# Nick-qsv/MLP-PPO-2PLY-MULTI

Measured on AMD Instinct MI355X. Metric: self-play env steps/sec (whole node) at 1-ply and 2-ply, 1/2/4/8 MI355X, higher is better.
Workload: dtype u8 game state + fp16x2-split MFMA (fp32 acc); 1 GPU; 8192 game lanes per GPU (8192 total), 1-ply softmax select (configs[3]/[4] lane shard: 65,536 lanes at N=8); lanes_per_gpu=8192, lanes_total=8192, ply=1, harvest_every=300, engine=fused step kernel, lockstep launches (reproducible: --dump-outputs), parallelism=single GPU

## Files before the change

### mlp-ppo-2ply-multi_amd/csrc/bgx_fused.hip

```cpp
#define BGX_LANE_ID_AT_USE 1
#include "bgx_engine.h"
#include "bgx_mlp.h"
#include "bgx_movegen.h"

namespace bgx {

constexpr int PROF_STRIDE = 128;

template <int FL> struct FusedTail {
    uint4 lut[256];
    float w2s[128];
    int cnt[FL];
    int go[2];
    int qn[2];
    int ncl;
    unsigned tdone[64];
    unsigned chosen[FL];
    unsigned claim[FL];
    int pre[FL + 1];
    uint32_t job[FL][8];
    DrawSlot draw[FL];
    LaneState st[FL];
};
template <int FL> struct FCfg {
    static constexpr int NW = 12;
    static constexpr int WPE = NW / 4;
    static constexpr int P1_S = 256, P1_F = 160, P1_PF = 416;
    static constexpr int SL1 = 64 * 4 + 2 * P1_PF * 4;
    static constexpr int F_SCR = NW * SL1 > Slice<S_T2>::bytes ? NW * SL1 : Slice<S_T2>::bytes;
    static constexpr int F_W = F_SCR;
    static constexpr int CP_F = 128 * NW;
    static_assert(sizeof(CoopPathLds<NW, CP_F>) <= F_SCR, "path expansion fits the scratch");
    static constexpr int F_TAIL = F_W + NFRAG * 16;
    static constexpr int XS_FIT = (160 * 1024 - F_TAIL - (int)sizeof(FusedTail<FL>)) / (FL * 4);
    static constexpr int XS = XS_FIT < 96 ? XS_FIT : 96;
    static constexpr int LDS = F_TAIL + (int)sizeof(FusedTail<FL>) + FL * XS * 4;
    static_assert(XS >= 24 && LDS <= 160 * 1024, "fits the CU's LDS");
};

__device__ __forceinline__ const FusedArgs& launch_args() {
    auto p = __builtin_amdgcn_kernarg_segment_ptr();
    asm volatile("" : "+s"(p));
    return *(const FusedArgs*)p;
}
__device__ __forceinline__ MovegenArgs job_args(const FusedArgs& f) {
    MovegenArgs a{};
    a.out_mode = OUT_PACKED_SLOT;
    a.cap = f.cap;
    a.out_packed = f.cand;
    a.out_count = const_cast<int32_t*>(f.e.cand_cnt);
    a.ws_global = f.ws_global;
    a.ws_slots = f.ws_slots;
    a.ws_words_per_wave = f.ws_words_per_block;
    a.force_tier = f.force_tier;
    a.err_flags = f.e.err_flags;
    return a;
}

template <bool PROF, int FL>
__global__ __launch_bounds__(64 * FCfg<FL>::NW, FCfg<FL>::WPE) void fused_step_kernel(FusedArgs) {
    using C = FCfg<FL>;
    constexpr int NW = C::NW, SL1 = C::SL1, F_W = C::F_W, F_TAIL = C::F_TAIL, XS = C::XS;
    constexpr int P1_S = C::P1_S, P1_F = C::P1_F, P1_PF = C::P1_PF;
    constexpr int CP_F = C::CP_F;
    constexpr bool PAIR = FL == 32;
    constexpr int NT = 64 * NW;
    extern __shared__ __attribute__((aligned(16))) unsigned long long smem[];
    uint8_t* lds = (uint8_t*)smem;
    FusedTail<FL>& T = *(FusedTail<FL>*)(lds + F_TAIL);
    float* xs = (float*)(lds + F_TAIL + sizeof(FusedTail<FL>));
    const int t = (int)threadIdx.x, w = t >> 6, l = lane_id();
    {
        const FusedArgs& f = launch_args();
        for (int i = t; i < 256; i += NT) T.lut[i] = lut_entry((uint32_t)i, f.feat_scale);
        for (int i = t; i < 128; i += NT) T.w2s[i] = f.rowc[i];
    }
    for (int i = t; i < 64; i += NT) T.tdone[i] = 0u;
    for (int i = t; i < FL; i += NT) T.chosen[i] = T.claim[i] = 0u;
    unsigned qtag = 0u;
    uint4* wl = (uint4*)(lds + F_W);
    static_assert(NFRAG % 64 == 0, "W fragments in whole wave chunks");
    {
        const uint4* const wsrc = launch_args().wfrag;
        for (int c = w; c < NFRAG / 64; c += NW)
            __builtin_amdgcn_global_load_lds((__attribute__((address_space(1))) void*)(void*)(wsrc + 64 * c + l),
                                             (__attribute__((address_space(3))) void*)(void*)(wl + 64 * c), 16, 0, 0);
    }
    const uint4* wf = wl;

    unsigned long long n_rows = 0, n_fb = 0, n_steps = 0;
    const unsigned long long wg_begin = PROF ? wall_clock64() : 0ull;
    const unsigned long long cyc_begin = PROF ? __builtin_amdgcn_s_memtime() : 0ull;
    unsigned long long t_loop0 = 0, t_loop1 = 0;
    unsigned long long t_step = 0, late_sum = 0, late_n = 0;
    int step_idx = 0;
    unsigned long long ph[6] = {0, 0, 0, 0, 0, 0}, tc = 0, tw[4] = {0, 0, 0, 0}, t2c = 0, t3n = 0;
    unsigned long long tjd[4] = {0, 0, 0, 0};
    unsigned long long tcs[3] = {0, 0, 0};
    unsigned long long tdr[3] = {0, 0, 0};
    unsigned long long tms[3] = {0, 0, 0};
    unsigned long long tpr[7] = {0, 0, 0, 0, 0, 0, 0};
    constexpr bool prof = PROF;
    auto tick = [&](int k) {
        if (prof && t == 0) {
            const unsigned long long c = wall_clock64();
            ph[k] += c - tc;
            tc = c;
        }
    };
    const int groups = (launch_args().e.L + FL - 1) / FL;
    uint32_t* const slw = (uint32_t*)(lds + (size_t)w * SL1);
    Mem M1 = slice_mem<P1_S, P1_F, P1_PF>(slw);
    asm volatile("s_waitcnt vmcnt(0)" ::: "memory");
    for (int g = (int)blockIdx.x; g < groups; g += (int)gridDim.x) {
        int nlive, n_iter;
        bool t1_ready;
        {
            const FusedArgs& f = launch_args();
            nlive = f.e.L - g * FL < FL ? f.e.L - g * FL : FL;
            n_iter = f.budget > 0 ? f.n_cap : f.n_steps;
            t1_ready = f.t1_ready != 0;
            for (int v = t; v < nlive; v += NT) {
                lane_load(f.e, g * FL + v, T.st[v]);
                if (t1_ready) T.cnt[v] = f.t1cnt[g * FL + v];
            }
        }
        if (t1_ready) {
            __syncthreads();
            for (int q = t; q < nlive * 8; q += NT) {
                const int v = q >> 3, k = q & 7;
                const LaneState& st = T.st[v];
                T.job[v][k] = k < 7 ? st.w[k] : (uint32_t)st.p | ((uint32_t)st.d0 << 8) | ((uint32_t)st.d1 << 16);
            }
        }
        auto ticket = [&](int s) -> int {
            const FusedArgs& f = launch_args();
            const int full = nlive << 8;
            if (f.budget <= 0) return s < f.n_steps ? full : 0;
            if (s >= f.n_cap) return 0;
            const unsigned long long old = atomicAdd(f.budget_ctr, (unsigned long long)nlive);
            return old < (unsigned long long)f.budget ? full : 0;
        };
        auto wait_flag = [&](const unsigned* fl) {
            for (unsigned spin = 0; __hip_atomic_load(fl, __ATOMIC_RELAXED, __HIP_MEMORY_SCOPE_WORKGROUP) != qtag;
                 ++spin) {
                if (spin >= (1u << 24)) {
                    if (l == 0) atomicOr(launch_args().e.err_flags, BGX_ERRF_WAIT_BOUND);
                    break;
                }
                __builtin_amdgcn_s_sleep(1);
            }
        };
        if (prof && t == 0 && !t_loop0) t_loop0 = wall_clock64();
        for (int step = -1; step < n_iter; ++step) {
            int nr = 0;
            const int gv = step >= 0 ? T.go[step & 1] : nlive << 8;
            if (!gv) break;
            const int lo = gv & 255, hi = gv >> 8;
            const auto act = [&](int v) { return v >= lo && v < hi; };
            if (prof && t == 0) tc = wall_clock64();
            if (step >= 0) {
                n_steps += (unsigned long long)(hi - lo);
                const int cnt_l = act(l) ? T.cnt[l] : 0;
                uint32_t ovf = (uint32_t)ballot(l < FL && cnt_l < 0);
                while (ovf) {
                    const int v = __ffs(ovf) - 1;
                    ovf &= ovf - 1u;
                    ++n_fb;
                    const unsigned long long c2 = prof ? wall_clock64() : 0ull;
                    const int j = g * FL + v;
                    const uint32_t* q = T.job[v];
                    const JobIn in = make_job(q[0], q[1], q[2], q[3], q[4], q[5], q[6], (int)(q[7] & 255u),
                                              (int)((q[7] >> 8) & 255u), (int)(q[7] >> 16));
                    const FusedArgs& f = launch_args();
                    const MovegenArgs a = job_args(f);
                    FlatCursor fc;
                    auto run_global = [&]() -> int {
                        uint32_t* base = f.ws_global + (size_t)blockIdx.x * f.ws_words_per_block;
                        const Mem G = global_mem(base, f.ws_slots);
                        st32<true>(G.map + l, 0u);
                        sync<true>();
                        if (prof) ++t3n;
                        const int r = run_job<true>(a, j, in, G, fc);
                        if (r < 0 && l == 0) atomicOr(a.err_flags, BGX_ERRF_FALLBACK_OVERFLOW);
                        return r < 0 ? 0 : r;
                    };
                    int r2 = -1;
                    if (in.d0 == in.d1 && doubles_by_path(in.R) && f.force_tier < 3) {
                        auto& C = *(CoopPathLds<NW, CP_F>*)lds;
                        uint32_t* fin = nullptr;
                        r2 = coop_doubles_path<NW, CP_F>(in, C, fin);
                        if (r2 >= 0) {
                            emit_records<false>(a, j, in, fin, r2, 0, 64 * w, 64 * NW);
                            if (t == 0) {
                                T.cnt[v] = r2;
                                a.out_count[j] = r2;
                            }
                        }
                        __syncthreads();
                    }
                    if (r2 < 0 && w == 0) {
                        const Mem M2 = lds_mem<S_T2>(smem);
                        int r = f.force_tier >= 3 ? -1 : run_job<false>(a, j, in, M2, fc);
                        if (r < 0) r = run_global();
                        if (l == 0) T.cnt[v] = r;
                    }
                    __syncthreads();
                    if (prof) t2c += wall_clock64() - c2;
                }
                const int c = act(l) ? T.cnt[l] : 0;
                const int cap = launch_args().cap;
                const int rows = l < FL && c > 0 ? 1 + (c < cap ? c : cap) : 0;
                const int incl = wave_incl_scan(rows);
                if (l <= FL) T.pre[l] = incl - rows;
                wave_sync();
                nr = T.pre[FL];
                n_rows += (unsigned long long)nr;
                tick(1);
            }
            const int n_tiles = (nr + 31) >> 5;
            const int np = step >= 0 ? (hi - lo + 1) >> 1 : 0;
            if (t == 0) {
                T.qn[0] = NW;
                T.qn[1] = NW;
                T.ncl = 0;
            }
            ++qtag;
            M1.map[l] = 0u;
            wave_sync();
            __syncthreads();
            const int nj = step >= 0 || !t1_ready ? hi - lo : 0;
            const bool dbl = act(l) && T.st[l].d0 == T.st[l].d1;
            const uint32_t dmask = (uint32_t)ballot(dbl), omask = (uint32_t)ballot(act(l) && !dbl);
            const int nd = __popc(dmask);
            auto lane_of = [&](int r) -> int {
                int v = 0;
#pragma unroll
                for (int sstep = FL / 2; sstep >= 1; sstep >>= 1)
                    if (T.pre[v + sstep] <= r) v += sstep;
                return v;
            };
            const unsigned long long m0 = prof ? wall_clock64() : 0ull;
            const bool one = n_tiles <= 64;
            const int npass = one ? 1 : 3;
            for (int pass = 0; pass < npass; ++pass) {
                const int qt = one || pass == 0 ? n_tiles : 0;
                const int qp = one || pass == 1 ? np : 0;
                const int qj = one || pass == 2 ? nj : 0;
                const bool pipelined = one && np > 0;
                int* qc = &T.qn[pass & 1];
                const int qd = pass == npass - 1 ? 1 : 0;
                int it = w;
                while (it < qt + qp + qj + qd) {
                    if (it < qt) {
                        const unsigned long long i0 = prof ? wall_clock64() : 0ull;
                        const FusedArgs& f = launch_args();
                        const uint32_t* const k_rows = f.e.rows;
                        const uint32_t* const k_cand = f.cand;
                        float* const k_vbuf = f.vbuf;
                        const int k_cap = f.cap;
                        const float k_b2 = f.b2, k_fs = f.feat_scale;
                        const int r = it * 32 + (l & 31);
                        uint4 bx = make_uint4(0, 0, 0, 0), by = make_uint4(0, 0, 0, 0);
                        int vl = 0, k = 0;
                        if (r < nr) {
                            vl = lane_of(r);
                            k = r - T.pre[vl];
                            const int li = g * FL + vl;
                            const uint32_t* src =
                                k == 0 ? k_rows + (size_t)li * 8 : k_cand + ((size_t)li * k_cap + (k - 1)) * 8;
                            bx = ((const uint4*)src)[0];
                            by = ((const uint4*)src)[1];
                        }
                        unsigned long long i1 = 0, i2 = 0;
                        if (prof) {
                            __builtin_amdgcn_s_waitcnt(0);
                            i1 = wall_clock64();
                            tms[0] += i1 - i0;
                        }
                        const float v = mlp_tile4<PROF>(wf, T.lut, T.w2s, k_fs, bx, by, &i2);
                        if (prof) {
                            const float vv = __shfl(v, 0);
                            asm volatile("" ::"v"(vv));
                            const unsigned long long i3 = wall_clock64();
                            tms[1] += i2 - i1;
                            tms[2] += i3 - i2;
                        }
                        if (l < 32 && r < nr) {
                            const float val = v + k_b2;
                            if (k < XS) xs[vl * XS + k] = val;
                            else k_vbuf[(size_t)(g * FL + vl) * (k_cap + 1) + k] = val;
                        }
                        __builtin_amdgcn_fence(__ATOMIC_RELEASE, "workgroup");
                        if (l == 0) __hip_atomic_store(&T.tdone[it & 63], qtag, __ATOMIC_RELAXED, __HIP_MEMORY_SCOPE_WORKGROUP);
                        if (prof) tw[1] += wall_clock64() - i0;
                    } else if (it < qt + qp) {
                        const int p = it - qt;
                        const FusedArgs& f = launch_args();
                        const EngineDev& e = f.e;
                        if (pipelined) {
                            const int va = lo + 2 * p, vb = lo + 2 * p + 2 < hi ? lo + 2 * p + 2 : hi;
                            const int r0 = T.pre[va], r1 = T.pre[vb];
                            if (r1 > r0) {
                                for (int tt = r0 >> 5; tt <= (r1 - 1) >> 5; ++tt) wait_flag(&T.tdone[tt]);
                                __builtin_amdgcn_fence(__ATOMIC_ACQUIRE, "workgroup");
                            }
                        }
                        const int v = lo + 2 * p + (l >> 5);
                        const bool lead = (l & 31) == 0;
                        if (v < hi) {
                            const int i = g * FL + v;
                            const unsigned long long s1 = prof ? wall_clock64() : 0ull;
                            LaneState sr = T.st[v];
                            const int n_full = T.cnt[v];
                            const int n = n_full < e.max_legal ? n_full : e.max_legal;
                            SlotRng rng;
                            rng.seed = e.seed;
                            rng.gid = (uint32_t)(e.lane_base + i);
                            rng.dt = lane_dice(e, i);
                            rng.load(T.draw[v], sr.ctr);
                            unsigned long long c0 = 0;
                            if (prof) {
                                __builtin_amdgcn_s_waitcnt(0);
                                c0 = wall_clock64();
                                tcs[0] += c0 - s1;
                            }
                            if (n <= 0) {
                                lane_advance(e, i, sr, rng, -1, sr.w, 0.0f, 0.0f, 0, lead);
                            } else {
                                const float* xv = xs + v * XS;
                                const float* vv = f.vbuf + (size_t)i * (f.cap + 1);
                                const float Tm = e.temperature;
                                const float u = rng.uniform01();
                                const int pick =
                                    n + 1 <= XS
                                        ? pick_action_half([&](int kk) { return xv[1 + kk] / Tm; }, n, e.greedy != 0, u)
                                        : pick_action_half(
                                              [&](int kk) { return (1 + kk < XS ? xv[1 + kk] : vv[1 + kk]) / Tm; }, n,
                                              e.greedy != 0, u);
                                if (prof) {
                                    const unsigned long long c1 = wall_clock64();
                                    tw[2] += c1 - s1;
                                    tcs[1] += c1 - c0;
                                    c0 = c1;
                                }
                                uint32_t nb[8];
                                load_packed(f.cand + ((size_t)i * f.cap + pick) * 8, nb);
                                const float va = 1 + pick < XS ? xv[1 + pick] : vv[1 + pick];
                                lane_advance(e, i, sr, rng, pick, nb, xv[0], va, n_full, lead);
                                if (prof) {
                                    __builtin_amdgcn_s_waitcnt(0);
                                    tcs[2] += wall_clock64() - c0;
                                }
                            }
                            wave_sync();
                            if (lead) T.st[v] = sr;
                            if (prof) tw[3] += wall_clock64() - s1;
                        }
                        __builtin_amdgcn_fence(__ATOMIC_RELEASE, "workgroup");
                        if (lead && v < hi)
                            __hip_atomic_store(&T.chosen[v], qtag, __ATOMIC_RELAXED, __HIP_MEMORY_SCOPE_WORKGROUP);
                    } else if (it < qt + qp + qj) {
                        const int kj = it - qt - qp;
                        const FusedArgs& f = launch_args();
                        const MovegenArgs a = job_args(f);
                        const bool k_pair = f.pair != 0;
                        int v, v2 = -1;
                        if (pipelined) {
                            v = -1;
                            for (unsigned spin = 0; v < 0; ++spin) {
                                const bool ready =
                                    act(l) &&
                                    __hip_atomic_load(&T.chosen[l], __ATOMIC_RELAXED, __HIP_MEMORY_SCOPE_WORKGROUP) == qtag &&
                                    __hip_atomic_load(&T.claim[l], __ATOMIC_RELAXED, __HIP_MEMORY_SCOPE_WORKGROUP) != qtag;
                                __builtin_amdgcn_fence(__ATOMIC_ACQUIRE, "workgroup");
                                const bool isd = ready && T.st[l].d0 == T.st[l].d1;
                                const uint32_t md = (uint32_t)ballot(isd), mo = (uint32_t)ballot(ready && !isd);
                                if (md | mo) {
                                    const int cand = md ? __ffs(md) - 1 : __ffs(mo) - 1;
                                    int won = 0;
                                    if (l == 0) {
                                        const unsigned old = T.claim[cand];
                                        won = old != qtag && atomicCAS(&T.claim[cand], old, qtag) == old;
                                        if (PAIR && won) atomicAdd(&T.ncl, 1);
                                    }
                                    if (uniform(won)) v = cand;
                                    if (prof && v >= 0) tpr[2] += 1;
                                } else {
                                    if (PAIR &&
                                        uniform(__hip_atomic_load(&T.ncl, __ATOMIC_RELAXED, __HIP_MEMORY_SCOPE_WORKGROUP)) >= nj)
                                        break;
                                    if (spin >= (1u << 24)) {
                                        if (l == 0) atomicOr(a.err_flags, BGX_ERRF_WAIT_BOUND);
                                        v = kj;
                                        break;
                                    }
                                    __builtin_amdgcn_s_sleep(1);
                                }
                            }
                        } else {
                            v = kj < nd ? select_bit(dmask, kj) : select_bit(omask, kj - nd);
                        }
                        if (PAIR && pipelined && v >= 0 && (k_pair || prof) && T.st[v].d0 != T.st[v].d1) {
                            const bool free_l =
                                act(l) &&
                                __hip_atomic_load(&T.chosen[l], __ATOMIC_RELAXED, __HIP_MEMORY_SCOPE_WORKGROUP) == qtag &&
                                __hip_atomic_load(&T.claim[l], __ATOMIC_RELAXED, __HIP_MEMORY_SCOPE_WORKGROUP) != qtag;
                            __builtin_amdgcn_fence(__ATOMIC_ACQUIRE, "workgroup");
                            const bool cls = (free_l || l == v) && T.st[l].d0 != T.st[l].d1 &&
                                             nd_by_rule(make_root(T.st[l].w, (int)T.st[l].p));
                            const uint32_t mc = (uint32_t)ballot(cls);
                            uint32_t mf = mc & ~(1u << v);
                            if ((mc >> v) & 1u) {
                                if (prof) {
                                    tpr[3] += 1;
                                    if (mf) tpr[4] += 1;
                                }
                                for (int att = 0; att < 2 && mf && v2 < 0 && k_pair; ++att) {
                                    const int c2 = __ffs(mf) - 1;
                                    mf &= mf - 1u;
                                    int won2 = 0;
                                    if (l == 0) {
                                        const unsigned old = T.claim[c2];
                                        won2 = old != qtag && atomicCAS(&T.claim[c2], old, qtag) == old;
                                        if (won2) atomicAdd(&T.ncl, 1);
                                    }
                                    if (uniform(won2)) v2 = c2;
                                }
                            }
                        }
                        const unsigned long long q0 = prof ? wall_clock64() : 0ull;
                        bool paired = false;
                        if (PAIR && v2 >= 0) {
                            if (l < 16) {
                                const int vq = l < 8 ? v : v2, k = l & 7;
                                const LaneState& sq = T.st[vq];
                                T.job[vq][k] =
                                    k < 7 ? sq.w[k] : (uint32_t)sq.p | ((uint32_t)sq.d0 << 8) | ((uint32_t)sq.d1 << 16);
                            }
                            wave_sync();
                            int na = 0, nb = 0;
                            paired = a.force_tier < 2 &&
                                     job_records_pair<false>(a, g * FL + v, T.job[v], g * FL + v2, T.job[v2], M1, na, nb);
                            wave_sync();
                            if (paired && l == 0) {
                                T.cnt[v] = na;
                                T.cnt[v2] = nb;
                            }
                            if (prof && paired) {
                                tpr[5] += wall_clock64() - q0;
                                tpr[6] += 1;
                            }
                        }
                        const int nv = !PAIR ? 1 : (v < 0 ? 0 : (v2 >= 0 ? 2 : 1));
                        for (int q = 0; q < nv; ++q) {
                            const int vq = q ? v2 : v;
                            const unsigned long long q1 = prof ? wall_clock64() : 0ull;
                            const LaneState& st = T.st[vq];
                            if (l < 8)
                                T.job[vq][l] =
                                    l < 7 ? st.w[l] : (uint32_t)st.p | ((uint32_t)st.d0 << 8) | ((uint32_t)st.d1 << 16);
                            if (paired) continue;
                            const JobIn in =
                                make_job(st.w[0], st.w[1], st.w[2], st.w[3], st.w[4], st.w[5], st.w[6], st.p, st.d0, st.d1);
                            int rule2 = 0;
                            uint32_t* fin = nullptr;
                            const int nf = a.force_tier >= 2
                                               ? -1
                                               : job_records<false>(in, M1, fin, prof ? &rule2 : nullptr);
                            if (nf >= 0) emit_records<false>(a, g * FL + vq, in, fin, nf, 0);
                            wave_sync();
                            if (l == 0) T.cnt[vq] = nf;
                            if (prof) {
                                const int kd = in.d0 == in.d1 ? 0 : 2;
                                tjd[kd] += wall_clock64() - q1;
                                tjd[kd + 1] += 1;
                                if (rule2) {
                                    tpr[0] += wall_clock64() - q1;
                                    tpr[1] += 1;
                                }
                            }
                        }
                    } else {
                        const unsigned long long d0 = prof ? wall_clock64() : 0ull;
                        const FusedArgs& f = launch_args();
                        const int ld = lane_id();
                        const int v = ld & (FL - 1), k = ld / FL;
                        const bool mine = k < 2 && act(v);
                        if (pipelined) {
                            for (unsigned spin = 0;; ++spin) {
                                const bool pend =
                                    mine &&
                                    __hip_atomic_load(&T.chosen[v], __ATOMIC_RELAXED, __HIP_MEMORY_SCOPE_WORKGROUP) != qtag;
                                if (!ballot(pend)) break;
                                if (spin >= (1u << 24)) {
                                    if (l == 0) atomicOr(f.e.err_flags, BGX_ERRF_WAIT_BOUND);
                                    break;
                                }
                                __builtin_amdgcn_s_sleep(1);
                            }
                            __builtin_amdgcn_fence(__ATOMIC_ACQUIRE, "workgroup");
                        }
                        const unsigned long long d1 = prof ? wall_clock64() : 0ull;
                        if (mine)
                            draw_fill(T.draw[v], f.e.seed, (uint32_t)(f.e.lane_base + g * FL + v), T.st[v].ctr, k);
                        if (prof) {
                            __builtin_amdgcn_s_waitcnt(0);
                            tdr[0] += wall_clock64() - d0;
                            tdr[1] += d1 - d0;
                            tdr[2] += 1;
                        }
                    }
                    int kn = 0;
                    if (l == 0) kn = atomicAdd(qc, 1);
                    it = uniform(kn);
                }
                if (pass + 1 < npass) {
                    if (t == 0) T.qn[(pass + 1) & 1] = NW;
                    __syncthreads();
                }
            }
            if (prof) tw[0] += wall_clock64() - m0;
            tick(3);
            if (t == 0) T.go[(step + 1) & 1] = ticket(step + 1);
            __syncthreads();
            tick(4);
            if (prof && t == 0 && step >= 0) ph[5] += 1;
            if (prof && t == 0) {
                const unsigned long long c = wall_clock64();
                if (step >= 0) {
                    if (step_idx < 24) {
                        unsigned long long* const pr = launch_args().prof;
                        atomicAdd(pr + (size_t)blockIdx.x * PROF_STRIDE + 32 + step_idx, c - t_step);
                        atomicAdd(pr + (size_t)blockIdx.x * PROF_STRIDE + 64 + step_idx, 1ull);
                    }
                    else { late_sum += c - t_step; ++late_n; }
                    ++step_idx;
                }
                t_step = c;
            }
        }
        if (prof && t == 0) t_loop1 = wall_clock64();
        const FusedArgs& f = launch_args();
        const EngineDev& e = f.e;
        for (int v = t; v < nlive; v += NT) {
            lane_store(e, g * FL + v, T.st[v]);
            f.t1cnt[g * FL + v] = T.cnt[v];
        }
        if (f.hv_hdr) {
            uint32_t* hs = (uint32_t*)lds;
            if (w == 0) {
                int ne = 0, nr = 0;
                bool lost = false;
                if (l < nlive) {
                    const LaneState& s = T.st[l];
                    ne = (int)(s.epi - s.hepi);
                    nr = (int)(s.ep_first - s.harv);
                    lost = ne > e.HR || nr > e.R;
                }
                if (lost) ne = nr = 0;
                const int ie = wave_incl_scan(ne), ir = wave_incl_scan(nr);
                const uint32_t te = (uint32_t)__shfl(ie, 63), tr = (uint32_t)__shfl(ir, 63);
                if (l < FL) {
                    hs[l] = (uint32_t)(ie - ne);
                    hs[64 + l] = (uint32_t)(ir - nr);
                }
                if (l == 0) {
                    unsigned long long base = 0ull;
                    uint32_t fit = 1u;
                    if (te | tr) {
                        const unsigned long long add = ((unsigned long long)te << 32) | tr;
                        base = atomicAdd(f.hv_ctr, add);
                        fit = (base >> 32) + te <= (unsigned long long)f.hv_ep_cap &&
                              (base & 0xFFFFFFFFull) + tr <= (unsigned long long)f.hv_rec_cap;
                        if (fit) atomicAdd(f.hv_commit, add);
                    }
                    hs[128] = te;
                    hs[129] = tr;
                    hs[130] = (uint32_t)(base >> 32);
                    hs[131] = (uint32_t)base;
                    hs[132] = fit;
                }
                if (l < FL) hs[136 + l] = lost ? 1u : 0u;
            }
            __syncthreads();
            const uint32_t te = hs[128], tr = hs[129], be = hs[130], br = hs[131], fit = hs[132];
            auto owner = [&](const uint32_t* pre, uint32_t k) -> int {
                int v = 0;
#pragma unroll
                for (int sstep = FL / 2; sstep >= 1; sstep >>= 1)
                    if (pre[v + sstep] <= k) v += sstep;
                return v;
            };
            if (fit) {
                for (uint32_t q = (uint32_t)t; q < 4u * te; q += NT) {
                    const uint32_t k = q >> 2;
                    const int v = owner(hs, k);
                    const uint32_t ep = T.st[v].hepi + (k - hs[v]);
                    const uint4* src = (const uint4*)(e.hring + ((size_t)(g * FL + v) * e.HR + (ep & (uint32_t)(e.HR - 1))) *
                                                                    EP_WORDS);
                    ((uint4*)(f.hv_hdr + (size_t)(be + k) * EP_WORDS))[q & 3u] = src[q & 3u];
                }
                for (uint32_t q = (uint32_t)t; q < 3u * tr; q += NT) {
                    const uint32_t r = q / 3u, c = q - 3u * r;
                    const int v = owner(hs + 64, r);
                    const uint32_t rr = T.st[v].harv + (r - hs[64 + v]);
                    const uint4* src =
                        (const uint4*)(e.ring + ((size_t)(g * FL + v) * e.R + (rr & (uint32_t)(e.R - 1))) * REC_WORDS);
                    ((uint4*)(f.hv_rec + (size_t)(br + r) * REC_WORDS))[c] = src[c];
                }
            }
            for (int v = t; v < nlive; v += NT) {
                if (fit || hs[136 + v]) {
                    e.harv[g * FL + v] = T.st[v].ep_first;
                    e.hepi[g * FL + v] = T.st[v].epi;
                }
            }
        }
        __syncthreads();
    }
    const FusedArgs& f = launch_args();
    const EngineDev& e = f.e;
    if (prof) {
        unsigned long long* P = f.prof + (size_t)blockIdx.x * PROF_STRIDE;
        if (t == 0) {
            P[24] = wg_begin;
            P[25] = wall_clock64();
            P[26] = n_rows;
            P[27] = n_fb;
            P[28] = n_steps;
            P[19] = t_loop0;
            P[20] = t_loop1;
            P[21] = __builtin_amdgcn_s_memtime() - cyc_begin;
            for (int k = 0; k < 6; ++k) atomicAdd(P + k, ph[k]);
            atomicAdd(P + 11, t2c);
            atomicAdd(P + 12, n_fb);
            atomicAdd(P + 13, t3n);
            atomicAdd(P + 18, (unsigned long long)NW * ph[5]);
            atomicAdd(P + 56, late_sum);
            atomicAdd(P + 57, late_n);
        }
        if (l == 0) {
            for (int k = 0; k < 4; ++k) atomicAdd(P + 7 + k, tw[k]);
            for (int k = 0; k < 4; ++k) atomicAdd(P + 14 + k, tjd[k]);
            for (int k = 0; k < 3; ++k) atomicAdd(P + 29 + k, tcs[k]);
            atomicAdd(P + 6, tms[0]);
            atomicAdd(P + 22, tms[1]);
            atomicAdd(P + 23, tms[2]);
            for (int k = 0; k < 7; ++k) atomicAdd(P + 88 + k, tpr[k]);
            for (int k = 0; k < 3; ++k) atomicAdd(P + 95 + k, tdr[k]);
        }
    }
    if (t == 0) {
        atomicAdd(e.stats + 0, n_steps);
        atomicAdd(e.stats + 3, n_rows);
        atomicAdd(e.stats + 4, n_steps);
        atomicAdd(e.stats + 5, n_fb);
        if (f.budget > 0 || f.hv_hdr) {
            __builtin_amdgcn_fence(__ATOMIC_RELEASE, "agent");
            if (atomicAdd(f.done_ctr, 1ull) == (unsigned long long)gridDim.x - 1ull) {
                __builtin_amdgcn_fence(__ATOMIC_ACQUIRE, "agent");
                if (f.budget > 0) __hip_atomic_store(f.budget_ctr, 0ull, __ATOMIC_RELAXED, __HIP_MEMORY_SCOPE_AGENT);
                if (f.hv_hdr) {
                    const unsigned long long c = __hip_atomic_load(f.hv_commit, __ATOMIC_RELAXED, __HIP_MEMORY_SCOPE_AGENT);
                    const uint32_t fl = atomicExch(e.err_flags, 0u) | (uint32_t)*f.hv_flags;
                    *f.hv_flags = fl;
                    *f.hv_next_flags = 0ull;
                    const uint32_t v[4] = {(uint32_t)(c >> 32), (uint32_t)c, fl, (uint32_t)(c >> 32)};
#pragma unroll
                    for (int k = 0; k < 4; ++k) {
                        f.hv_info[k] = v[k];
                        if (f.hv_hinfo) f.hv_hinfo[k] = v[k];
                    }
                    __hip_atomic_store(f.hv_next, 0ull, __ATOMIC_RELAXED, __HIP_MEMORY_SCOPE_AGENT);
                    __hip_atomic_store(f.hv_next_commit, 0ull, __ATOMIC_RELAXED, __HIP_MEMORY_SCOPE_AGENT);
                }
                __hip_atomic_store(f.done_ctr, 0ull, __ATOMIC_RELAXED, __HIP_MEMORY_SCOPE_AGENT);
            }
        }
    }
}

}

#ifdef BGX_STAMP
extern "C" int bgx_diag_stamps(unsigned long long* out32) {
    static unsigned long long h[256 * 32];
    if (hipMemcpyFromSymbol(h, HIP_SYMBOL(bgx::bgx_stamp_acc), sizeof(h)) != hipSuccess) return -1;
    for (int k = 0; k < 32; ++k) {
        out32[k] = 0;
        for (int b = 0; b < 256; ++b) out32[k] += h[b * 32 + k];
    }
    static unsigned long long z[256 * 32];
    return hipMemcpyToSymbol(HIP_SYMBOL(bgx::bgx_stamp_acc), z, sizeof(z)) == hipSuccess ? 0 : -1;
}
#endif

extern "C" hipError_t bgx_launch_fused(const bgx::FusedArgs* args, hipStream_t stream) {
    static int n_cu_dev[64] = {0};
    int cur = 0;
    if (hipGetDevice(&cur) != hipSuccess || cur < 0 || cur >= 64) cur = 0;
    int& n_cu = n_cu_dev[cur];
    if (!n_cu) {
        if (hipDeviceGetAttribute(&n_cu, hipDeviceAttributeMultiprocessorCount, cur) != hipSuccess || n_cu <= 0)
            n_cu = 256;
        const void* k16[] = {(const void*)bgx::fused_step_kernel<false, 16>, (const void*)bgx::fused_step_kernel<true, 16>};
        const void* k32[] = {(const void*)bgx::fused_step_kernel<false, 32>, (const void*)bgx::fused_step_kernel<true, 32>};
        for (const void* k : k16)
            if (hipFuncSetAttribute(k, hipFuncAttributeMaxDynamicSharedMemorySize, bgx::FCfg<16>::LDS) != hipSuccess)
                return hipErrorInvalidValue;
        for (const void* k : k32)
            if (hipFuncSetAttribute(k, hipFuncAttributeMaxDynamicSharedMemorySize, bgx::FCfg<32>::LDS) != hipSuccess)
                return hipErrorInvalidValue;
    }
    if (args->n_steps <= 0 || args->e.L <= 0) return hipSuccess;
    if (args->cap < 1 || args->cap > 2048) return hipErrorInvalidValue;
    const int L = args->e.L;
    const int fl = args->lanes_per_wg == 16 || args->lanes_per_wg == 32 ? args->lanes_per_wg
                   : ((L + 31) / 32 >= n_cu ? 32 : 16);
    const int groups = (L + fl - 1) / fl;
    int blocks = groups < n_cu ? groups : n_cu;
    if (blocks > args->ws_blocks) blocks = args->ws_blocks;
    const dim3 g(blocks), b(64 * (fl == 32 ? bgx::FCfg<32>::NW : bgx::FCfg<16>::NW));
    bgx::FusedArgs a = *args;
    if (a.budget > 0 && (groups > blocks || !a.budget_ctr || a.n_cap < a.n_steps)) a.budget = 0;
    if (fl == 32) {
        if (a.prof)
            hipLaunchKernelGGL((bgx::fused_step_kernel<true, 32>), g, b, bgx::FCfg<32>::LDS, stream, a);
        else
            hipLaunchKernelGGL((bgx::fused_step_kernel<false, 32>), g, b, bgx::FCfg<32>::LDS, stream, a);
    } else {
        if (a.prof)
            hipLaunchKernelGGL((bgx::fused_step_kernel<true, 16>), g, b, bgx::FCfg<16>::LDS, stream, a);
        else
            hipLaunchKernelGGL((bgx::fused_step_kernel<false, 16>), g, b, bgx::FCfg<16>::LDS, stream, a);
    }
    return hipGetLastError();
}
```

### mlp-ppo-2ply-multi_amd/csrc/bgx_host_prof.cpp

```cpp
#include "bgx_prof.h"

#include <algorithm>
#include <utility>
#include <vector>

void fused_prof_report(const unsigned long long* p, int n_slots, FILE* out, const char* dump_path) {
    constexpr size_t W = kProfSlotWords;
    double s[W] = {0};
    for (int b = 0; b < n_slots; ++b)
        for (size_t k = 0; k < W; ++k) s[k] += (double)p[(size_t)b * W + k];
    const double n = s[5] > 0 ? s[5] : 1;
    const double nws = s[18] > 0 ? s[18] : 1;
    fprintf(out, "[bgx fused prof] us per workgroup step: tier2 + prefix %.2f, queue %.2f, end barrier %.2f "
            "(%.0f workgroup steps)\n", s[1] / n / 100, s[3] / n / 100, s[4] / n / 100, n);
    fprintf(out, "[bgx fused prof] wave-us per workgroup step in items: MLP tiles %.2f, choice pairs %.2f, "
            "tier-1 jobs %.2f (%.2f per wave-step of %d waves)\n", s[8] / n / 100, s[10] / n / 100,
            (s[14] + s[16]) / n / 100, (s[8] + s[10] + s[14] + s[16]) / nws / 100, (int)(nws / n + 0.5));
    fprintf(out, "[bgx fused prof] choice per wave-step: state + Philox refill %.2f, pick %.2f, "
            "env step %.2f us\n", s[29] / nws / 100, s[30] / nws / 100, s[31] / nws / 100);
    fprintf(out, "[bgx fused prof] draw item: %.2f us each, %.2f of it waiting for the choices (%.0f items, "
            "%.2f per workgroup step)\n", s[95] / (s[97] > 0 ? s[97] : 1) / 100,
            s[96] / (s[97] > 0 ? s[97] : 1) / 100, s[97], s[97] / n);
    fprintf(out, "[bgx fused prof] MLP tiles per workgroup step: rows + k mask %.2f, MFMA chain issue %.2f, "
            "drain + epilogue %.2f wave-us\n", s[6] / n / 100, s[22] / n / 100, s[23] / n / 100);
    fprintf(out, "[bgx fused prof] step us by index in the launch (workgroup-steps):");
    for (int k = 0; k < 24; ++k)
        fprintf(out, " %.2f (%.0f)", s[64 + k] > 0 ? s[32 + k] / s[64 + k] / 100 : 0.0, s[64 + k]);
    fprintf(out, "; later steps %.2f (%.0f)\n", s[57] > 0 ? s[56] / s[57] / 100 : 0.0, s[57]);
    fprintf(out, "[bgx fused prof] tier-2 jobs %.0f (%.0f reached tier 3), %.1f us each\n", s[12], s[13],
            s[11] / (s[12] > 0 ? s[12] : 1) / 100);
    fprintf(out, "[bgx fused prof] tier-1 job: doubles %.2f us (%.0f jobs), non-doubles %.2f us (%.0f jobs)\n",
            s[14] / (s[15] > 0 ? s[15] : 1) / 100, s[15], s[16] / (s[17] > 0 ? s[17] : 1) / 100, s[17]);
    const double items = s[8] + s[10] + s[14] + s[16] + s[93];
    fprintf(out, "[bgx fused prof] tier-1 rule-mode two-move job: %.2f us (%.0f jobs), %.2f wave-us per workgroup "
            "step, %.1f %% of the item wave-us\n", s[88] / (s[89] > 0 ? s[89] : 1) / 100, s[89], s[88] / n / 100,
            100.0 * s[88] / (items > 0 ? items : 1));
    fprintf(out, "[bgx fused prof] pipelined job claims %.0f: %.0f of a rule-mode non-doubles lane, %.0f of them "
            "(%.1f %%) with a second such lane ready and unclaimed\n", s[90], s[91], s[92],
            100.0 * s[92] / (s[91] > 0 ? s[91] : 1));
    fprintf(out, "[bgx fused prof] tier-1 pair items: %.0f pairs formed (%.2f per workgroup step), %.2f us each, "
            "%.2f wave-us per workgroup step\n", s[94], s[94] / n, s[93] / (s[94] > 0 ? s[94] : 1) / 100,
            s[93] / n / 100);
    std::vector<std::pair<double, int>> dur;
    unsigned long long b_min = ~0ull, b_max = 0, e_max = 0;
    for (int b = 0; b < n_slots; ++b) {
        const unsigned long long* q = &p[(size_t)b * W];
        if (q[25] <= q[24]) continue;
        dur.push_back({(double)(q[25] - q[24]) / 100.0, b});
        b_min = q[24] < b_min ? q[24] : b_min;
        b_max = q[24] > b_max ? q[24] : b_max;
        e_max = q[25] > e_max ? q[25] : e_max;
    }
    if (dump_path) {
        if (FILE* fp = fopen(dump_path, "w")) {
            fprintf(fp, "wg,begin,end,loop0,loop1,rows,tier2,lane_steps\n");
            for (int b = 0; b < n_slots; ++b) {
                const unsigned long long* q = &p[(size_t)b * W];
                if (q[25] <= q[24]) continue;
                fprintf(fp, "%d,%llu,%llu,%llu,%llu,%llu,%llu,%llu\n", b, q[24], q[25], q[19], q[20], q[26],
                        q[27], q[28]);
            }
            fclose(fp);
        }
    }
    if (!dur.empty()) {
        std::sort(dur.begin(), dur.end());
        double mean = 0;
        for (auto& d : dur) mean += d.first;
        mean /= (double)dur.size();
        const size_t nd = dur.size();
        const unsigned long long* qm = &p[(size_t)dur[nd / 2].second * W];
        const unsigned long long* qx = &p[(size_t)dur[nd - 1].second * W];
        fprintf(out, "[bgx fused prof] last launch, %zu workgroups: duration us min %.1f p50 %.1f mean %.1f "
                "p90 %.1f max %.1f; begin skew %.1f us, span %.1f us; lane-steps %llu; rows / tier-2 jobs: "
                "median workgroup %llu / %llu, slowest %llu / %llu\n",
                nd, dur[0].first, dur[nd / 2].first, mean, dur[(nd * 9) / 10].first, dur[nd - 1].first,
                (double)(b_max - b_min) / 100.0, (double)(e_max - b_min) / 100.0, qx[28], qm[26], qm[27],
                qx[26], qx[27]);
        std::vector<double> pro, loop, epi, mhz;
        for (auto& d : dur) {
            const unsigned long long* q = &p[(size_t)d.second * W];
            if (q[19] < q[24] || q[20] < q[19] || q[25] < q[20]) continue;
            pro.push_back((double)(q[19] - q[24]) / 100.0);
            loop.push_back((double)(q[20] - q[19]) / 100.0);
            epi.push_back((double)(q[25] - q[20]) / 100.0);
            mhz.push_back((double)q[21] / ((double)(q[25] - q[24]) / 100.0));
        }
        if (!pro.empty()) {
            auto med = [](std::vector<double>& v) {
                std::sort(v.begin(), v.end());
                return v[v.size() / 2];
            };
            fprintf(out, "[bgx fused prof] last launch shape (median workgroup): prologue %.1f us, step loop "
                    "%.1f us, epilogue %.1f us; shader clock %.0f MHz\n", med(pro), med(loop), med(epi),
                    med(mhz));
        }
    }
}
```

Baseline: 290.0 million env_steps/s.

## Replace per-lane claim arrays with packed 64-bit bitmask claim words

Replaces the per-lane chosen/claim tag arrays and the ncl counter with two 64-bit LDS words. One word packs an open mask and a stepped mask, the other packs doubles and rule classes. Job waves claim lanes with a single fetch_and on the open mask and find pair partners from the class bits, instead of polling every lane's tags and resolving ownership with CAS. The goal is to cut LDS polling, ballots and CAS contention in the pipelined job dispatch. It also adds profiling counters for the wait phases, and the ordering and termination logic is now a hand-written lock-free protocol.

Measured after the change: 308.2 million env_steps/s, median of 6. +6.3%, better.

```diff
diff --git a/mlp-ppo-2ply-multi_amd/csrc/bgx_claim.h b/mlp-ppo-2ply-multi_amd/csrc/bgx_claim.h
--- /dev/null
+++ b/mlp-ppo-2ply-multi_amd/csrc/bgx_claim.h
@@ -0,0 +1,106 @@
+#pragma once
+
+#include <cstdint>
+
+#ifndef BGX_CLAIM_FN
+#define BGX_CLAIM_FN inline
+#endif
+
+namespace bgx {
+
+struct alignas(16) ClaimWords {
+    unsigned long long so;
+    unsigned long long cls;
+};
+
+constexpr unsigned CLAIM_POLL_BOUND = 1u << 24;
+constexpr unsigned CLAIM_BOUND = 1u;
+constexpr unsigned CLAIM_RULE = 2u;
+constexpr unsigned CLAIM_PARTNER = 4u;
+
+struct Claim {
+    int v, v2;
+    unsigned flags;
+};
+
+BGX_CLAIM_FN uint32_t claim_range(int lo, int hi) {
+    return (hi >= 32 ? 0xFFFFFFFFu : (1u << hi) - 1u) & ~((1u << lo) - 1u);
+}
+BGX_CLAIM_FN int claim_bit_index(uint32_t bit) { return __builtin_ctz(bit); }
+
+template <class A> BGX_CLAIM_FN void claim_publish_class(A& a, ClaimWords& W, int v, bool dbl, bool rule) {
+    const unsigned long long bit = 1ull << v;
+    const unsigned long long c = (dbl ? bit : 0ull) | (rule ? bit << 32 : 0ull);
+    if (c) a.or_relaxed(&W.cls, c);
+}
+template <class A> BGX_CLAIM_FN void claim_publish_open(A& a, ClaimWords& W, int v) {
+    const unsigned long long bit = 1ull << v;
+    a.or_release(&W.so, bit | (bit << 32));
+}
+
+template <bool PAIR, class A>
+BGX_CLAIM_FN Claim claim_take(A& a, ClaimWords& W, uint32_t range, bool pair_on, bool survey) {
+    Claim r{-1, -1, 0u};
+    for (unsigned spin = 0;; ++spin) {
+        unsigned long long so, cls;
+        a.load2(W, so, cls);
+        uint32_t open = (uint32_t)so;
+        while (open) {
+            const uint32_t md = open & (uint32_t)cls, pick = md ? md : open;
+            const uint32_t bit = pick & (0u - pick);
+            const unsigned long long old = a.fetch_and(&W.so, ~(unsigned long long)bit);
+            so = old & ~(unsigned long long)bit;
+            if (old & bit) {
+                r.v = claim_bit_index(bit);
+                break;
+            }
+            open = (uint32_t)so;
+        }
+        if (r.v >= 0) {
+            if (PAIR && (pair_on || survey)) {
+                const uint32_t rule = (uint32_t)(cls >> 32), bit = 1u << r.v;
+                if (rule & bit) {
+                    r.flags |= CLAIM_RULE;
+                    uint32_t mf = (uint32_t)so & rule & ~bit;
+                    if (mf) r.flags |= CLAIM_PARTNER;
+                    for (int att = 0; att < 2 && mf && pair_on; ++att) {
+                        const uint32_t b2 = mf & (0u - mf);
+                        const unsigned long long old = a.fetch_and(&W.so, ~(unsigned long long)b2);
+                        if (old & b2) {
+                            r.v2 = claim_bit_index(b2);
+                            break;
+                        }
+                        mf = (uint32_t)old & rule & ~bit & ~b2;
+                    }
+                }
+            }
+            a.acquire();
+            return r;
+        }
+        if ((uint32_t)(so >> 32) == range) {
+            const unsigned long long chk = a.load(&W.so);
+            if ((uint32_t)(chk >> 32) == range && (uint32_t)chk == 0u) return r;
+            if ((uint32_t)chk) continue;
+        }
+        if (spin >= CLAIM_POLL_BOUND) {
+            r.flags |= CLAIM_BOUND;
+            return r;
+        }
+        a.relax();
+    }
+}
+
+template <class A> BGX_CLAIM_FN bool claim_wait_stepped(A& a, const ClaimWords& W, uint32_t range) {
+    bool ok = true;
+    for (unsigned spin = 0; ((uint32_t)(a.load(&W.so) >> 32) & range) != range; ++spin) {
+        if (spin >= CLAIM_POLL_BOUND) {
+            ok = false;
+            break;
+        }
+        a.relax();
+    }
+    a.acquire();
+    return ok;
+}
+
+}
diff --git a/mlp-ppo-2ply-multi_amd/csrc/bgx_fused.hip b/mlp-ppo-2ply-multi_amd/csrc/bgx_fused.hip
--- a/mlp-ppo-2ply-multi_amd/csrc/bgx_fused.hip
+++ b/mlp-ppo-2ply-multi_amd/csrc/bgx_fused.hip
@@ -2,6 +2,8 @@
 #include "bgx_engine.h"
 #include "bgx_mlp.h"
 #include "bgx_movegen.h"
+#define BGX_CLAIM_FN BGX_DEV
+#include "bgx_claim.h"
 
 namespace bgx {
 
@@ -13,10 +15,8 @@
     int cnt[FL];
     int go[2];
     int qn[2];
-    int ncl;
+    ClaimWords cw;
     unsigned tdone[64];
-    unsigned chosen[FL];
-    unsigned claim[FL];
     int pre[FL + 1];
     uint32_t job[FL][8];
     DrawSlot draw[FL];
@@ -43,6 +43,46 @@
     asm volatile("" : "+s"(p));
     return *(const FusedArgs*)p;
 }
+struct WaveClaimOps {
+    int l;
+    static __device__ __forceinline__ unsigned long long uni64(unsigned long long x) {
+        const uint32_t a = (uint32_t)__builtin_amdgcn_readfirstlane((int)(uint32_t)x);
+        const uint32_t b = (uint32_t)__builtin_amdgcn_readfirstlane((int)(uint32_t)(x >> 32));
+        return (unsigned long long)a | ((unsigned long long)b << 32);
+    }
+    __device__ __forceinline__ unsigned long long load(const unsigned long long* p) const {
+        return uni64(__hip_atomic_load(p, __ATOMIC_RELAXED, __HIP_MEMORY_SCOPE_WORKGROUP));
+    }
+    __device__ __forceinline__ void load2(const ClaimWords& W, unsigned long long& so, unsigned long long& cls) const {
+        typedef uint32_t v4u __attribute__((ext_vector_type(4)));
+        const v4u r = *(const volatile __attribute__((address_space(3))) v4u*)(const void*)&W;
+        so = uni64((unsigned long long)r.x | ((unsigned long long)r.y << 32));
+        cls = uni64((unsigned long long)r.z | ((unsigned long long)r.w << 32));
+    }
+    __device__ __forceinline__ unsigned long long fetch_and(unsigned long long* p, unsigned long long m) const {
+        unsigned long long old = 0ull;
+        if (l == 0) old = __hip_atomic_fetch_and(p, m, __ATOMIC_RELAXED, __HIP_MEMORY_SCOPE_WORKGROUP);
+        return uni64(old);
+    }
+    __device__ __forceinline__ void or_relaxed(unsigned long long* p, unsigned long long m) const {
+        __hip_atomic_fetch_or(p, m, __ATOMIC_RELAXED, __HIP_MEMORY_SCOPE_WORKGROUP);
+    }
+    __device__ __forceinline__ void or_release(unsigned long long* p, unsigned long long m) const {
+        __hip_atomic_fetch_or(p, m, __ATOMIC_RELEASE, __HIP_MEMORY_SCOPE_WORKGROUP);
+    }
+    __device__ __forceinline__ void acquire() const { __builtin_amdgcn_fence(__ATOMIC_ACQUIRE, "workgroup"); }
+    __device__ __forceinline__ void relax() const { __builtin_amdgcn_s_sleep(1); }
+};
+__device__ __forceinline__ bool lane_by_rule(const LaneState& s) {
+    const bool p1 = s.p != 0;
+    Root R{};
+    R.player = s.p;
+    R.m0 = p1 ? s.w[3] : s.w[0];
+    R.m2 = p1 ? s.w[5] : s.w[2];
+    R.bar = (p1 ? s.w[6] >> 4 : s.w[6]) & 15u;
+    R.off = (p1 ? s.w[6] >> 12 : s.w[6] >> 8) & 15u;
+    return nd_by_rule(R);
+}
 __device__ __forceinline__ MovegenArgs job_args(const FusedArgs& f) {
     MovegenArgs a{};
     a.out_mode = OUT_PACKED_SLOT;
@@ -76,7 +116,6 @@
         for (int i = t; i < 128; i += NT) T.w2s[i] = f.rowc[i];
     }
     for (int i = t; i < 64; i += NT) T.tdone[i] = 0u;
-    for (int i = t; i < FL; i += NT) T.chosen[i] = T.claim[i] = 0u;
     unsigned qtag = 0u;
     uint4* wl = (uint4*)(lds + F_W);
     static_assert(NFRAG % 64 == 0, "W fragments in whole wave chunks");
@@ -100,6 +139,7 @@
     unsigned long long tdr[3] = {0, 0, 0};
     unsigned long long tms[3] = {0, 0, 0};
     unsigned long long tpr[7] = {0, 0, 0, 0, 0, 0, 0};
+    unsigned long long twt[3] = {0, 0, 0};
     constexpr bool prof = PROF;
     auto tick = [&](int k) {
         if (prof && t == 0) {
@@ -223,7 +263,8 @@
             if (t == 0) {
                 T.qn[0] = NW;
                 T.qn[1] = NW;
-                T.ncl = 0;
+                T.cw.so = 0ull;
+                T.cw.cls = 0ull;
             }
             ++qtag;
             M1.map[l] = 0u;
@@ -299,15 +340,18 @@
                         const FusedArgs& f = launch_args();
                         const EngineDev& e = f.e;
                         if (pipelined) {
+                            const unsigned long long w0 = prof ? wall_clock64() : 0ull;
                             const int va = lo + 2 * p, vb = lo + 2 * p + 2 < hi ? lo + 2 * p + 2 : hi;
                             const int r0 = T.pre[va], r1 = T.pre[vb];
                             if (r1 > r0) {
                                 for (int tt = r0 >> 5; tt <= (r1 - 1) >> 5; ++tt) wait_flag(&T.tdone[tt]);
                                 __builtin_amdgcn_fence(__ATOMIC_ACQUIRE, "workgroup");
                             }
+                            if (prof) twt[0] += wall_clock64() - w0;
                         }
                         const int v = lo + 2 * p + (l >> 5);
                         const bool lead = (l & 31) == 0;
+                        const WaveClaimOps cops{l};
                         if (v < hi) {
                             const int i = g * FL + v;
                             const unsigned long long s1 = prof ? wall_clock64() : 0ull;
@@ -354,12 +398,16 @@
                                 }
                             }
                             wave_sync();
-                            if (lead) T.st[v] = sr;
+                            if (lead) {
+                                T.st[v] = sr;
+                                if (pipelined)
+                                    claim_publish_class(cops, T.cw, v, sr.d0 == sr.d1,
+                                                        PAIR && sr.d0 != sr.d1 && lane_by_rule(sr));
+                            }
                             if (prof) tw[3] += wall_clock64() - s1;
                         }
                         __builtin_amdgcn_fence(__ATOMIC_RELEASE, "workgroup");
-                        if (lead && v < hi)
-                            __hip_atomic_store(&T.chosen[v], qtag, __ATOMIC_RELAXED, __HIP_MEMORY_SCOPE_WORKGROUP);
+                        if (pipelined && lead && v < hi) claim_publish_open(cops, T.cw, v);
                     } else if (it < qt + qp + qj) {
                         const int kj = it - qt - qp;
                         const FusedArgs& f = launch_args();
@@ -367,67 +415,23 @@
                         const bool k_pair = f.pair != 0;
                         int v, v2 = -1;
                         if (pipelined) {
-                            v = -1;
-                            for (unsigned spin = 0; v < 0; ++spin) {
-                                const bool ready =
-                                    act(l) &&
-                                    __hip_atomic_load(&T.chosen[l], __ATOMIC_RELAXED, __HIP_MEMORY_SCOPE_WORKGROUP) == qtag &&
-                                    __hip_atomic_load(&T.claim[l], __ATOMIC_RELAXED, __HIP_MEMORY_SCOPE_WORKGROUP) != qtag;
-                                __builtin_amdgcn_fence(__ATOMIC_ACQUIRE, "workgroup");
-                                const bool isd = ready && T.st[l].d0 == T.st[l].d1;
-                                const uint32_t md = (uint32_t)ballot(isd), mo = (uint32_t)ballot(ready && !isd);
-                                if (md | mo) {
-                                    const int cand = md ? __ffs(md) - 1 : __ffs(mo) - 1;
-                                    int won = 0;
-                                    if (l == 0) {
-                                        const unsigned old = T.claim[cand];
-                                        won = old != qtag && atomicCAS(&T.claim[cand], old, qtag) == old;
-                                        if (PAIR && won) atomicAdd(&T.ncl, 1);
-                                    }
-                                    if (uniform(won)) v = cand;
-                                    if (prof && v >= 0) tpr[2] += 1;
-                                } else {
-                                    if (PAIR &&
-                                        uniform(__hip_atomic_load(&T.ncl, __ATOMIC_RELAXED, __HIP_MEMORY_SCOPE_WORKGROUP)) >= nj)
-                                        break;
-                                    if (spin >= (1u << 24)) {
-                                        if (l == 0) atomicOr(a.err_flags, BGX_ERRF_WAIT_BOUND);
-                                        v = kj;
-                                        break;
-                                    }
-                                    __builtin_amdgcn_s_sleep(1);
-                                }
+                            const unsigned long long c0 = prof ? wall_clock64() : 0ull;
+                            const WaveClaimOps cops{l};
+                            const Claim cl = claim_take<PAIR>(cops, T.cw, claim_range(lo, hi), k_pair, prof);
+                            v = cl.v;
+                            v2 = cl.v2;
+                            if (cl.flags & CLAIM_BOUND) {
+                                if (l == 0) atomicOr(a.err_flags, BGX_ERRF_WAIT_BOUND);
+                                v = kj;
+                            }
+                            if (prof) {
+                                twt[1] += wall_clock64() - c0;
+                                if (cl.v >= 0) tpr[2] += 1;
+                                if (cl.flags & CLAIM_RULE) tpr[3] += 1;
+                                if (cl.flags & CLAIM_PARTNER) tpr[4] += 1;
                             }
                         } else {
                             v = kj < nd ? select_bit(dmask, kj) : select_bit(omask, kj - nd);
-                        }
-                        if (PAIR && pipelined && v >= 0 && (k_pair || prof) && T.st[v].d0 != T.st[v].d1) {
-                            const bool free_l =
-                                act(l) &&
-                                __hip_atomic_load(&T.chosen[l], __ATOMIC_RELAXED, __HIP_MEMORY_SCOPE_WORKGROUP) == qtag &&
-                                __hip_atomic_load(&T.claim[l], __ATOMIC_RELAXED, __HIP_MEMORY_SCOPE_WORKGROUP) != qtag;
-                            __builtin_amdgcn_fence(__ATOMIC_ACQUIRE, "workgroup");
-                            const bool cls = (free_l || l == v) && T.st[l].d0 != T.st[l].d1 &&
-                                             nd_by_rule(make_root(T.st[l].w, (int)T.st[l].p));
-                            const uint32_t mc = (uint32_t)ballot(cls);
-                            uint32_t mf = mc & ~(1u << v);
-                            if ((mc >> v) & 1u) {
-                                if (prof) {
-                                    tpr[3] += 1;
-                                    if (mf) tpr[4] += 1;
-                                }
-                                for (int att = 0; att < 2 && mf && v2 < 0 && k_pair; ++att) {
-                                    const int c2 = __ffs(mf) - 1;
-                                    mf &= mf - 1u;
-                                    int won2 = 0;
-                                    if (l == 0) {
-                                        const unsigned old = T.claim[c2];
-                                        won2 = old != qtag && atomicCAS(&T.claim[c2], old, qtag) == old;
-                                        if (won2) atomicAdd(&T.ncl, 1);
-                                    }
-                                    if (uniform(won2)) v2 = c2;
-                                }
-                            }
                         }
                         const unsigned long long q0 = prof ? wall_clock64() : 0ull;
                         bool paired = false;
@@ -452,7 +456,7 @@
                                 tpr[6] += 1;
                             }
                         }
-                        const int nv = !PAIR ? 1 : (v < 0 ? 0 : (v2 >= 0 ? 2 : 1));
+                        const int nv = v < 0 ? 0 : (PAIR && v2 >= 0 ? 2 : 1);
                         for (int q = 0; q < nv; ++q) {
                             const int vq = q ? v2 : v;
                             const unsigned long long q1 = prof ? wall_clock64() : 0ull;
@@ -488,18 +492,9 @@
                         const int v = ld & (FL - 1), k = ld / FL;
                         const bool mine = k < 2 && act(v);
                         if (pipelined) {
-                            for (unsigned spin = 0;; ++spin) {
-                                const bool pend =
-                                    mine &&
-                                    __hip_atomic_load(&T.chosen[v], __ATOMIC_RELAXED, __HIP_MEMORY_SCOPE_WORKGROUP) != qtag;
-                                if (!ballot(pend)) break;
-                                if (spin >= (1u << 24)) {
-                                    if (l == 0) atomicOr(f.e.err_flags, BGX_ERRF_WAIT_BOUND);
-                                    break;
-                                }
-                                __builtin_amdgcn_s_sleep(1);
-                            }
-                            __builtin_amdgcn_fence(__ATOMIC_ACQUIRE, "workgroup");
+                            const WaveClaimOps cops{l};
+                            if (!claim_wait_stepped(cops, T.cw, claim_range(lo, hi)) && l == 0)
+                                atomicOr(f.e.err_flags, BGX_ERRF_WAIT_BOUND);
                         }
                         const unsigned long long d1 = prof ? wall_clock64() : 0ull;
                         if (mine)
@@ -520,10 +515,12 @@
                     __syncthreads();
                 }
             }
-            if (prof) tw[0] += wall_clock64() - m0;
+            const unsigned long long m1 = prof ? wall_clock64() : 0ull;
+            if (prof) tw[0] += m1 - m0;
             tick(3);
             if (t == 0) T.go[(step + 1) & 1] = ticket(step + 1);
             __syncthreads();
+            if (prof) twt[2] += wall_clock64() - m1;
             tick(4);
             if (prof && t == 0 && step >= 0) ph[5] += 1;
             if (prof && t == 0) {
@@ -649,6 +646,7 @@
             atomicAdd(P + 23, tms[2]);
             for (int k = 0; k < 7; ++k) atomicAdd(P + 88 + k, tpr[k]);
             for (int k = 0; k < 3; ++k) atomicAdd(P + 95 + k, tdr[k]);
+            for (int k = 0; k < 3; ++k) atomicAdd(P + 98 + k, twt[k]);
         }
     }
     if (t == 0) {
diff --git a/mlp-ppo-2ply-multi_amd/csrc/bgx_host_prof.cpp b/mlp-ppo-2ply-multi_amd/csrc/bgx_host_prof.cpp
--- a/mlp-ppo-2ply-multi_amd/csrc/bgx_host_prof.cpp
+++ b/mlp-ppo-2ply-multi_amd/csrc/bgx_host_prof.cpp
@@ -41,6 +41,9 @@
     fprintf(out, "[bgx fused prof] tier-1 pair items: %.0f pairs formed (%.2f per workgroup step), %.2f us each, "
             "%.2f wave-us per workgroup step\n", s[94], s[94] / n, s[93] / (s[94] > 0 ? s[94] : 1) / 100,
             s[93] / n / 100);
+    fprintf(out, "[bgx fused prof] waits per wave-step: choice tile wait %.2f, job claim %.2f, end barrier %.2f us "
+            "(%.2f, %.2f, %.2f wave-us per workgroup step)\n", s[98] / nws / 100, s[99] / nws / 100,
+            s[100] / nws / 100, s[98] / n / 100, s[99] / n / 100, s[100] / n / 100);
     std::vector<std::pair<double, int>> dur;
     unsigned long long b_min = ~0ull, b_max = 0, e_max = 0;
     for (int b = 0; b < n_slots; ++b) {
```
